# NYXFLOWER/GripNet

Hardware: NVIDIA B200
Metric: GripNet fwd+bwd edges/sec per epoch (pose-0 shape) (higher is better)
Workload: dtype f32

## Files before the change

gripnet_b200/_lib.py:

```python
import ctypes as C
import os

_HERE = os.path.dirname(os.path.abspath(__file__))
LIB_PATH = os.path.join(_HERE, "libgripnet_b200.so")


class GripnetLibraryError(RuntimeError):
    pass


class GnCsr(C.Structure):
    _fields_ = [
        ("n_rows", C.c_int32), ("n_cols", C.c_int32), ("nnz", C.c_int32), ("chunk_len", C.c_int32),
        ("n_chunks", C.c_int32), ("flags", C.c_int32),
        ("rowptr", C.c_void_p), ("col", C.c_void_p), ("val", C.c_void_p),
        ("chunk_ptr", C.c_void_p), ("chunk_row", C.c_void_p), ("chunk_beg", C.c_void_p),
        ("row_counter", C.c_void_p),
    ]


class GnAdamTensor(C.Structure):
    _fields_ = [("param", C.c_void_p), ("grad", C.c_void_p), ("exp_avg", C.c_void_p), ("exp_avg_sq", C.c_void_p),
                ("n", C.c_int64)]

# ... 5 lines not shown
class GnHaloPeer(C.Structure):
    _fields_ = [("idx", C.c_void_p), ("count", C.c_int64), ("dst_row", C.c_int64)]


class GnSumSegment(C.Structure):
    _fields_ = [("dst", C.c_void_p), ("n", C.c_int64), ("slot_offset", C.c_int64)]


_P, _I32, _I64, _F, _SZ, _INT = C.c_void_p, C.c_int32, C.c_int64, C.c_float, C.c_size_t, C.c_int
_CSR = C.POINTER(GnCsr)

SIGNATURES = {
    "gn_version": (_INT, []),
    "gn_error_string": (C.c_char_p, [_INT]),
    "gn_last_cuda_error": (_INT, []),
    "gn_last_cuda_error_string": (C.c_char_p, []),
    "gn_launch_count": (C.c_uint64, []),
    "gn_csr_from_keys_workspace_bytes": (_SZ, [_I64, _I32]),
    "gn_csr_from_keys": (_INT, [_P, _I64, _I32, _P, _P, _P, _SZ, _P]),
    "gn_rowptr_slice": (_INT, [_P, _I32, _I32, _P, _P]),
    "gn_build_chunks_workspace_bytes": (_SZ, [_I32]),
    "gn_build_chunks": (_INT, [_P, _I32, _I32, _P, _P, _P, _I64, _P, _P, _SZ, _P]),
    "gn_gcn_prep_workspace_bytes": (_SZ, [_I64, _I32, _I32]),
    "gn_gcn_prep": (_INT, [_P, _P, _P, _I64, _I32, _I32, _INT, _F, _P, _P, _P, _P, _P, _P, _P, _P, _P, _P, _P,
                           _P, _P, _P, _P, _SZ, _P]),
    "gn_edge_filter_workspace_bytes": (_SZ, [_I64]),
    "gn_edge_filter": (_INT, [_P, _P, _P, _I64, _INT, _I64, _I64, _P, _P, _P, _P, _I64, _P, _P, _SZ, _P]),
    "gn_gcn_part_workspace_bytes": (_SZ, [_I64, _I32]),
    "gn_gcn_part_structure": (_INT, [_P, _P, _P, _I64, _I32, _I32, _INT, _F, _P, _P, _P, _P, _P, _P, _P, _SZ, _P]),
    "gn_gcn_part_values": (_INT, [_P, _P, _I32, _I32, _P, _P, _INT, _P, _P]),
    "gn_rgcn_prep_workspace_bytes": (_SZ, [_I64, _I32, _I32]),
    "gn_rgcn_prep": (_INT, [_P, _P, _I64, _P, _I32, _I32, _P, _P, _P, _P, _P, _P, _P, _P, _P, _SZ, _P]),
    "gn_index_prep_workspace_bytes": (_SZ, [_I64, _I32]),
    "gn_index_prep": (_INT, [_P, _I64, _I32, _P, _P, _P, _SZ, _P]),
    "gn_spmm": (_INT, [_CSR, _P, _I64, _I32, _P, _P, _P, _I64, _INT, _P, _I64, _P, _P]),
    "gn_sgemm_workspace_bytes": (_SZ, [_I32, _I32, _I32, _I32, _INT]),
    "gn_sgemm": (_INT, [_INT, _INT, _I32, _I32, _I32, _P, _I64, _P, _I64, _P, _I64, _I32, _I64, _I64, _I64, _INT,
                        _F, _INT, _P, _I64, _P, _I64, _P, _I32, _P, _SZ, _P]),
    "gn_tc_gemm_workspace_bytes": (_SZ, [_I32, _I32, _I32]),
    "gn_tc_gemm": (_INT, [_INT, _I32, _I32, _I32, _P, _I64, _P, _I64, _P, _I64, _P, _I64, _P, _I64, _P, _SZ, _P]),
    "gn_tc_gemm_rel_workspace_bytes": (_SZ, [_I32, _I32, _I32, _I32]),
    "gn_tc_gemm_rel": (_INT, [_I32, _I32, _I32, _I32, _P, _I64, _P, _P, _I64, _P, _SZ, _P]),
    "gn_tc_rel_image": (_INT, [_I32, _I32, _I32, _I32, _P, _P, _SZ, _P]),
    "gn_tc_gemm_rel_image": (_INT, [_I32, _I32, _I32, _I32, _P, _I64, _P, _SZ, _P, _I64, _P]),
    "gn_tc_tn_workspace_bytes": (_SZ, [_I64, _I32, _I32]),
    "gn_tc_tn": (_INT, [_P, _I64, _P, _I64, _I64, _I32, _I32, _P, _I64, _I32, _I64, _P, _SZ, _P]),
    "gn_distmult_fwd": (_INT, [_P, _I64, _I32, _P, _P, _P, _P, _I64, _INT, _P, _P]),
    "gn_distmult_coef": (_INT, [_P, _P, _I64, _INT, _P, _P]),
    "gn_pair_prep_workspace_bytes": (_SZ, [_I64]),
    "gn_pair_prep": (_INT, [_P, _P, _P, _I64, _I32, _I32, _P, _P, _P, _P, _SZ, _P]),
    "gn_distmult_bwd_pairs": (_INT, [_CSR, _P, _P, _P, _P, _I64, _I32, _P, _P, _P]),
    "gn_distmult_grads_workspace_bytes": (_SZ, [_I32, _I32, _I32]),
    "gn_distmult_grads": (_INT, [_P, _P, _I32, _I32, _I32, _P, _I64, _P, _P, _I64, _P, _P, _SZ, _P]),
    "gn_softmax_fwd": (_INT, [_P, _I64, _I32, _P, _P]),
    "gn_softmax_bwd": (_INT, [_P, _P, _I64, _I32, _P, _P]),
    "gn_map2d": (_INT, [_INT, _P, _I64, _P, _I64, _I64, _I32, _P]),
    "gn_relu_bwd": (_INT, [_P, _I64, _P, _I64, _P, _I64, _I64, _I32, _P]),
    "gn_abs_bwd": (_INT, [_P, _I64, _P, _I64, _P, _I64, _I64, _I32, _F, _P]),
    "gn_axpby": (_INT, [_P, _I64, _F, _P, _I64, _F, _P, _I64, _I64, _I32, _P]),
    "gn_zero": (_INT, [_P, _SZ, _P]),
    "gn_mean3": (_INT, [_P, _I64, _P, _I64, _P, _I64, _P, _I64, _I64, _I32, _P]),
    "gn_colsum_workspace_bytes": (_SZ, [_I64, _I32]),
    "gn_colsum": (_INT, [_P, _I64, _I64, _I32, _P, _P, _SZ, _P]),
    "gn_loss_workspace_bytes": (_SZ, [_I64]),
    "gn_lp_loss_fwd": (_INT, [_P, _I64, _P, _I64, _F, _P, _P, _SZ, _P]),
    "gn_lp_loss_bwd": (_INT, [_P, _I64, _P, _I64, _F, _P, _P, _P, _P]),
    "gn_nc_loss_fwd": (_INT, [_P, _I64, _I32, _P, _F, _P, _P, _SZ, _P]),
    "gn_nc_loss_bwd": (_INT, [_P, _I64, _I32, _P, _F, _P, _P, _P]),
    "gn_negsample_table_bytes": (_SZ, [_I64]),
    "gn_negsample_build": (_INT, [_P, _P, _I64, _I64, _P, _I32, _P, _SZ, _P]),
    "gn_negsample_draw": (_INT, [_P, _SZ, _I64, _I64, _P, _I32, C.c_uint64, _P, _P, _P, _P]),
    "gn_adam_max_tensors_per_launch": (_INT, []),
    "gn_adam_step": (_INT, [_P, _I32, C.c_double, C.c_double, C.c_double, C.c_double, C.c_double, _P, _P]),
    "gn_lp_metrics_workspace_bytes": (_SZ, [_I64, _I64, _I32]),
    "gn_lp_metrics": (_INT, [_P, _I64, _P, _I64, _P, _P, _I32, _P, _P, _SZ, _P]),
    "gn_argmax_rows": (_INT, [_P, _I64, _I64, _I32, _P, _P]),
    "gn_nc_metrics_workspace_bytes": (_SZ, [_I32]),
    "gn_nc_metrics": (_INT, [_P, _P, _I64, _I32, _P, _P, _SZ, _P]),
    "gn_peer_max_world": (_INT, []),
    "gn_peer_allgather": (_INT, [_P, _I32, _I32, _I64, _I64, _I64, _I32, _P, _P, _P, _P]),
    "gn_peer_halo_grid": (_INT, []),
    "gn_peer_halo_push": (_INT, [_P, _I32, _I32, _I64, _I64, _P, _I32, _P, _I64, _I32, _P, _P, _P, _P]),
    "gn_peer_max_segments": (_INT, []),
    "gn_peer_push": (_INT, [_P, _I32, _I32, _I64, _I64, _P, _I32, _I64, _I32, _P, _P, _P, _P]),
    "gn_slot_sum": (_INT, [_P, _I32, _I64, _P, _I32, _P]),
}

GN_ERR_CUDA = -4
EW_COPY, EW_ABS, EW_RELU, EW_ADD = 0, 1, 2, 3
CSR_ROW_IS_CHUNK = 1

_lib = None


def load():
    global _lib
    if _lib is not None:
        return _lib
    if not os.path.isfile(LIB_PATH):
        raise GripnetLibraryError(
            f"{LIB_PATH} not found: build it with `python -m gripnet_b200.build` "
            "(nvcc, sm_100a).  gripnet_b200 has no CPU or PyTorch fallback.")
    try:
        lib = C.CDLL(LIB_PATH)
    except OSError as e:
        raise GripnetLibraryError(f"cannot load {LIB_PATH}: {e}") from e
# ... 19 lines not shown
```

gripnet_b200/csrc/decoder.cu:

```cuda
#include <cstdlib>

#include "rowsplit.cuh"
#include "sortkit.cuh"

namespace gn {

constexpr int kMaxNV = 8;

template <int LPE, int VEC>
__global__ void __launch_bounds__(256) distmult_fwd_kernel(const float* __restrict__ z, int64_t ldz, int D,
                                                           const float* __restrict__ w,
                                                           const int64_t* __restrict__ src,
                                                           const int64_t* __restrict__ dst,
                                                           const int64_t* __restrict__ etype, int64_t n_edges,
                                                           int sigmoid, float* __restrict__ out) {
  constexpr int EPI = 32 / LPE;
  const int lane = threadIdx.x & 31;
  const int slot = lane / LPE, fl = lane % LPE;
  const int64_t warp = (int64_t(blockIdx.x) * blockDim.x + threadIdx.x) >> 5;
  const int64_t n_warps = (int64_t(gridDim.x) * blockDim.x) >> 5;
  for (int64_t e0 = warp * EPI; e0 < n_edges; e0 += n_warps * EPI) {
    const int64_t e = e0 + slot;
    float s = 0.f;
    if (e < n_edges) {
// ... 112 lines not shown
}

template <int LPE, int VEC, int NV>
__global__ void __launch_bounds__(256) pair_walk_kernel(const gn_csr csr, const int32_t* __restrict__ ent_other,
                                                        const int32_t* __restrict__ ent_eid,
                                                        const float* __restrict__ coef, const float* __restrict__ z,
                                                        int64_t ldz, int D, float* __restrict__ T,
                                                        float* __restrict__ partial) {
  ChunkInfo ci;
  if (!chunk_info(csr, ci)) return;
  constexpr int EPI = 32 / LPE;
  const int lane = threadIdx.x & 31;
  const int slot = lane / LPE, fl = lane % LPE;
  Vec<VEC> acc[NV];
#pragma unroll
  for (int v = 0; v < NV; ++v)
#pragma unroll
    for (int i = 0; i < VEC; ++i) acc[v].v[i] = 0.f;
  for (int s0 = ci.beg + slot; s0 < ci.end; s0 += 2 * EPI) {
    const int s1 = s0 + EPI;
    const bool has1 = s1 < ci.end;
    const float* pa0 = z + int64_t(__ldg(ent_other + s0)) * ldz;
    const float* pa1 = has1 ? z + int64_t(__ldg(ent_other + s1)) * ldz : z;
    const float g0 = __ldg(coef + __ldg(ent_eid + s0));
    const float g1 = has1 ? __ldg(coef + __ldg(ent_eid + s1)) : 0.f;
    Vec<VEC> a0[NV], a1[NV];
#pragma unroll
    for (int v = 0; v < NV; ++v) {
      const int f = (v * LPE + fl) * VEC;
      if (f < D) {
        a0[v] = load_vec<VEC>(pa0 + f);
        a1[v] = load_vec<VEC>(pa1 + f);
      }
    }
#pragma unroll
    for (int v = 0; v < NV; ++v) {
      const int f = (v * LPE + fl) * VEC;
      if (f < D) {
#pragma unroll
        for (int i = 0; i < VEC; ++i) {
          acc[v].v[i] = fmaf(g0, a0[v].v[i], acc[v].v[i]);
          acc[v].v[i] = fmaf(g1, a1[v].v[i], acc[v].v[i]);
        }
      }
    }
  }
#pragma unroll
  for (int v = 0; v < NV; ++v) reduce_slots<LPE, VEC>(acc[v]);
  const int row = ci.row;
  auto emit = [&](int, int f, const Vec<VEC>& sum) { store_vec<VEC>(T + int64_t(row) * D + f, sum); };
  finish_row<LPE, VEC, NV>(csr, ci, acc, D, partial, emit);
}

template <int NV>
__global__ void __launch_bounds__(256, 4) pair_walk_batch_kernel(const gn_csr csr, const int32_t* __restrict__ ent_other,
                                                                 const int32_t* __restrict__ ent_eid,
                                                                 const float* __restrict__ coef,
                                                                 const float* __restrict__ z, int64_t ldz, int D,
                                                                 float* __restrict__ T, float* __restrict__ partial) {
  ChunkInfo ci;
  if (!chunk_info(csr, ci)) return;
  const int lane = threadIdx.x & 31;
  const int slot = lane >> 3, fl = lane & 7;
  const int D4 = D >> 2;
  const unsigned ldb = unsigned(ldz) * 4u;
  const float4* __restrict__ z4 = reinterpret_cast<const float4*>(z) + fl;
  bool ok[NV];
#pragma unroll
  for (int v = 0; v < NV; ++v) ok[v] = (v * 8 + fl) < D4;
  Vec<4> acc[NV];
#pragma unroll
  for (int v = 0; v < NV; ++v)
#pragma unroll
    for (int i = 0; i < 4; ++i) acc[v].v[i] = 0.f;
  for (int base = ci.beg; base < ci.end; base += 32) {
    const int mine = base + lane;
    int o = 0;
    float g = 0.f;
    if (mine < ci.end) {
      o = __ldg(ent_other + mine);
      g = __ldg(coef + __ldg(ent_eid + mine));
    }
    const int steps = min(8, (ci.end - base + 3) >> 2);
#pragma unroll 2
    for (int t = 0; t < steps; ++t) {
      const int from = t * 4 + slot;
      const int oo = __shfl_sync(kFull, o, from);
      const float gg = __shfl_sync(kFull, g, from);
      const float4* za = row_ptr(z4, oo, ldb);
#pragma unroll
      for (int v = 0; v < NV; ++v) {
        if (ok[v]) {
          const float4 a = __ldg(za + v * 8);
          acc[v].v[0] = fmaf(gg, a.x, acc[v].v[0]);
          acc[v].v[1] = fmaf(gg, a.y, acc[v].v[1]);
          acc[v].v[2] = fmaf(gg, a.z, acc[v].v[2]);
          acc[v].v[3] = fmaf(gg, a.w, acc[v].v[3]);
        }
      }
    }
  }
#pragma unroll
  for (int v = 0; v < NV; ++v) reduce_slots<8, 4>(acc[v]);
  const int row = ci.row;
  auto emit = [&](int, int f, const Vec<4>& sum) { store_vec<4>(T + int64_t(row) * D + f, sum); };
  finish_row<8, 4, NV>(csr, ci, acc, D, partial, emit);
}

constexpr int kGradThreads = 1024;
constexpr int kGradSlabNodes = 96;

__device__ __forceinline__ float grads_reduce_groups(float acc, int g, int G, int f, int D, float* red) {
  if (g < G && f < D) red[g * D + f] = acc;
  __syncthreads();
  float s = 0.f;
  if (g == 0 && f < D) {
    s = red[f];
    for (int k = 1; k < G; ++k) s += red[k * D + f];
  }
  __syncthreads();
  return s;
}

__global__ void __launch_bounds__(kGradThreads) distmult_grads_kernel(const float* __restrict__ T,
                                                                     const float* __restrict__ T2, int n_nodes,
                                                                     int n_rel, int D, const float* __restrict__ z,
                                                                     int64_t ldz, const float* __restrict__ w,
                                                                     float* __restrict__ dz, int64_t lddz,
                                                                     float* __restrict__ dw, int n_slabs,
                                                                     float* __restrict__ slab_part,
                                                                     unsigned int* __restrict__ slab_count) {
  extern __shared__ float red[];
  __shared__ int s_last;
  const int G = kGradThreads / D;
  const int g = int(threadIdx.x) / D, f = int(threadIdx.x) % D;
  const int n_dw_blocks = dw ? n_rel * n_slabs : 0;
  constexpr int kU = 8;
  if (int(blockIdx.x) >= n_dw_blocks) {
    const int row = int(blockIdx.x) - n_dw_blocks;
    if (dz == nullptr || row >= n_nodes) return;
    float acc = 0.f;
    if (g < G) {
      for (int i0 = g; i0 < n_rel; i0 += kU * G) {
        float tv[kU], ov[kU];
#pragma unroll
        for (int u = 0; u < kU; ++u) {
          const int i = i0 + u * G;
          tv[u] = ov[u] = 0.f;
          if (i < n_rel) {
            const int64_t t = (int64_t(row) * n_rel + i) * D + f;
            tv[u] = __ldg(T + t);
            if (T2) tv[u] += __ldg(T2 + t);
            ov[u] = __ldg(w + int64_t(i) * D + f);
          }
        }
#pragma unroll
        for (int u = 0; u < kU; ++u) acc = fmaf(tv[u], ov[u], acc);
      }
    }
// ... 397 lines not shown
  GN_PW_CASES(4, 4)
  GN_PW_CASE(8, 4, 3)
  GN_PW_CASES(32, 4)
  GN_PW_CASES(4, 1)
  GN_PW_CASES(32, 1)
#undef GN_PW_CASES
#undef GN_PW_CASE
  return GN_ERR_ARG;
}

static bool grads_vec_ok(int D, const float* T, const float* T2, const float* z, int64_t ldz, const float* w,
                         const float* dz, int64_t lddz, const float* dw) {
  return D % 4 == 0 && D <= 128 && ldz % 4 == 0 && lddz % 4 == 0 && aligned16(T) && (!T2 || aligned16(T2)) &&
         aligned16(z) && aligned16(w) && (!dz || aligned16(dz)) && (!dw || aligned16(dw));
}

size_t gn_distmult_grads_workspace_bytes(int32_t n_nodes, int32_t n_rel, int32_t D) {
  const size_t slabs = size_t(ceil_div(n_nodes > 0 ? n_nodes : 1, kGradSlabNodes));
  return align_up(size_t(n_rel > 0 ? n_rel : 1) * 4) + size_t(n_rel > 0 ? n_rel : 1) * slabs * size_t(D > 0 ? D : 1) * 4 + 256;
}

int gn_distmult_grads(const float* T, const float* T2, int32_t n_nodes, int32_t n_rel, int32_t D, const float* z,
                      int64_t ldz, const float* w, float* dz, int64_t lddz, float* dw, void* ws, size_t ws_bytes,
                      void* stream) {
  if (n_nodes <= 0 || n_rel <= 0 || D <= 0 || D > kGradThreads || !T || !z || !w || (!dz && !dw)) return GN_ERR_ARG;
  cudaStream_t st = as_stream(stream);
  const bool vec = grads_vec_ok(D, T, T2, z, ldz, w, dz, lddz, dw);
  const int n_slabs = int(ceil_div(n_nodes, vec ? kVSlab : kGradSlabNodes));
  unsigned int* count = nullptr;
  float* part = nullptr;
  if (dw && n_slabs > 1) {
    if (!ws || ws_bytes < gn_distmult_grads_workspace_bytes(n_nodes, n_rel, D)) return GN_ERR_WORKSPACE;
    count = static_cast<unsigned int*>(ws);
    part = reinterpret_cast<float*>(static_cast<char*>(ws) + align_up(size_t(n_rel) * 4));
    GN_LAUNCH(zero_u32_kernel, (unsigned)ceil_div(n_rel, 256), 256, 0, st, count, n_rel);
  }
  if (vec) {
    const int C4 = D / 4;
    const int GR = n_rel > 32 ? 8 : 1;
    const int nodes_per_cta = kVSub / GR;
    const int64_t blocks = int64_t(dw ? n_rel * n_slabs : 0) + (dz ? ceil_div(n_nodes, nodes_per_cta) : 0);
    GN_LAUNCH(distmult_grads_vec_kernel, (unsigned)blocks, C4 * kVSub, size_t(kVSub) * C4 * sizeof(float4), st, T, T2,
              n_nodes, n_rel, D, z, ldz, w, dz, lddz, dw, n_slabs, part, count, GR);
    return GN_OK;
  }
  const int G = kGradThreads / D;
  const size_t smem = size_t(G) * size_t(D) * sizeof(float);
  const int64_t blocks = int64_t(dw ? n_rel * n_slabs : 0) + (dz ? n_nodes : 0);
  GN_LAUNCH(distmult_grads_kernel, (unsigned)blocks, kGradThreads, smem, st, T, T2, n_nodes, n_rel, D, z, ldz, w, dz,
            lddz, dw, n_slabs, part, count);
  return GN_OK;
}

}
```

gripnet_b200/ops.py:

```python
import os
import weakref

import torch

from . import _lib, streams
from .graph import _ptr, _stream, _ws, require_cuda, validate_index

EPS = 1e-13


class M:
    __slots__ = ("t", "ptr", "ld", "n", "f")

    def __init__(self, t, col0=0, width=None):
        assert t.dim() == 2 and t.stride(1) == 1 and t.dtype == torch.float32
        self.t = t
        self.n = t.size(0)
        self.f = t.size(1) - col0 if width is None else width
        self.ld = t.stride(0) if t.size(0) > 1 else max(t.size(1), 1)
        self.ptr = t.data_ptr() + 4 * col0


def _as_rows(x, name):
    require_cuda(x, name)
# ... 704 lines not shown
        need = ctx.needs_input_grad[0] or ctx.needs_input_grad[1]
        br = streams.Branch()
        br_s = struct_branch if struct_branch is not None else streams.Branch(background=True)
        if need:
            with br_s(pos_index, neg_index, edge_type):
                pair_struct(neg_index, edge_type, z.size(0), r_loc)
                pair_struct(pos_index, edge_type, z.size(0), r_loc)
        with br(z, w, ni, et):
            neg = _distmult_fwd(z, w, ni, et, sigmoid)
        pos = _distmult_fwd(z, w, pi, et, sigmoid)
        br.join()
        if need and br_s._parent is None:
            ctx.struct_branch = br_s
        else:
            ctx.struct_branch = None
            br_s.join()
        ctx.sigmoid = bool(sigmoid)
        ctx.keys = (pos_index, neg_index, edge_type)
        ctx.key_versions = tuple(t._version for t in ctx.keys)
        ctx.rel = (int(rel_lo), r_loc, w_full.size(0))
        ctx.save_for_backward(z, w, pos, neg)
        return pos, neg

    @staticmethod
    def backward(ctx, g_pos, g_neg):
        from .graph import pair_struct
        z, w, pos, neg = ctx.saved_tensors
        pos_key, neg_key, et_key = ctx.keys
        _check_versions(ctx.keys, ctx.key_versions, "pos / neg edge_index or edge_type")
        rel_lo, r, r_full = ctx.rel
        n = z.size(0)
        if ctx.struct_branch is not None:
            ctx.struct_branch.join()
            ctx.struct_branch = None
        ps_p = pair_struct(pos_key, et_key, n, r)
        ps_n = pair_struct(neg_key, et_key, n, r)
        g_pos, g_neg = g_pos.contiguous(), g_neg.contiguous()
        br = streams.Branch(enabled=ps_p is not ps_n)
        with br(g_neg, neg, z):
            coef_n = _distmult_coef(g_neg, neg, ctx.sigmoid)
            t_n = _pair_walk(ps_n, coef_n, z)
        coef_p = _distmult_coef(g_pos, pos, ctx.sigmoid)
        t_p = _pair_walk(ps_p, coef_p, z)
        br.join()
        dz, dw = _distmult_grads(t_p, t_n, z, w, ctx.needs_input_grad[0], ctx.needs_input_grad[1])
        if dw is not None and r != r_full:
            dw_full = torch.empty((r_full, w.size(1)), dtype=torch.float32, device=w.device)
            _lib.check(_lib.load().gn_zero(dw_full.data_ptr(), dw_full.numel() * 4, _stream()), "gn_zero")
            map2d(_lib.EW_COPY, M(dw), M(dw_full[rel_lo: rel_lo + r]))
            dw = dw_full
        return dz, dw, None, None, None, None, None, None, None


class MultiClass(torch.autograd.Function):
    @staticmethod
    def forward(ctx, z, weight, node_list, softmax):
        lib = _lib.load()
        z = _as_rows(z, "z")
        w = _as_rows(weight, "weight").contiguous()
        require_cuda(node_list, "node_list", torch.int64)
        if w.size(0) != z.size(1):
            raise RuntimeError("decoder weight rows must equal the embedding width")
        validate_index(node_list, z.size(0), "node_list")
        idx = node_list.contiguous().view(-1)
        m, d, c = idx.numel(), z.size(1), w.size(1)
        dev = z.device
        logits = torch.empty((m, c), dtype=torch.float32, device=dev)
        sgemm(False, False, m, c, d, z.data_ptr(), z.stride(0) if z.size(0) > 1 else d, w.data_ptr(), c,
              logits.data_ptr(), c, dev, a_rows=idx)
        if softmax:
            out = torch.empty_like(logits)
            _lib.check(lib.gn_softmax_fwd(_ptr(logits), m, c, _ptr(out), _stream()), "gn_softmax_fwd")
        else:
            out = logits
        ctx.softmax = bool(softmax)
        ctx.key_tensor = node_list
        ctx.save_for_backward(z, w, out, idx)
        return out

    @staticmethod
    def backward(ctx, grad):
        from .graph import index_struct
        lib = _lib.load()
        z, w, out, idx = ctx.saved_tensors
        n, d, c, m = z.size(0), z.size(1), w.size(1), idx.numel()
        dev = z.device
        g = grad.contiguous()
        ldz = z.stride(0) if n > 1 else d
        if ctx.softmax:
            gl = torch.empty_like(g)
            _lib.check(lib.gn_softmax_bwd(_ptr(out), _ptr(g), m, c, _ptr(gl), _stream()), "gn_softmax_bwd")
        else:
            gl = g
        dz = dw = None
        if ctx.needs_input_grad[1]:
            dw = torch.empty((d, c), dtype=torch.float32, device=dev)
            sgemm(True, False, d, c, m, z.data_ptr(), ldz, gl.data_ptr(), c, dw.data_ptr(), c, dev, a_rows=idx)
        if ctx.needs_input_grad[0]:
            grows = torch.empty((max(m, 1), d), dtype=torch.float32, device=dev)
            sgemm(False, True, m, d, c, gl.data_ptr(), c, w.data_ptr(), c, grows.data_ptr(), d, dev)
            st = index_struct(ctx.key_tensor, n)
            dz = torch.empty((n, d), dtype=torch.float32, device=dev)
            spmm(st.csr, M(grows), M(dz), d)
        return dz, dw, None, None


class LinkPredLoss(torch.autograd.Function):
    @staticmethod
    def forward(ctx, pos, neg):
        lib = _lib.load()
        pos = require_cuda(pos, "pos_score", torch.float32).contiguous()
        neg = require_cuda(neg, "neg_score", torch.float32).contiguous()
        dev = pos.device
        loss = torch.empty(1, dtype=torch.float32, device=dev)
        n = max(pos.numel(), neg.numel())
        ws = _ws(lib.gn_loss_workspace_bytes(n), dev)
        _lib.check(lib.gn_lp_loss_fwd(_ptr(pos), pos.numel(), _ptr(neg), neg.numel(), EPS, _ptr(loss), _ptr(ws),
                                      ws.numel(), _stream()), "gn_lp_loss_fwd")
        ctx.save_for_backward(pos, neg)
        return loss.view(())

    @staticmethod
    def backward(ctx, grad):
        lib = _lib.load()
        pos, neg = ctx.saved_tensors
        g = grad.contiguous().view(1)
        gp, gn_ = torch.empty_like(pos), torch.empty_like(neg)
        _lib.check(lib.gn_lp_loss_bwd(_ptr(pos), pos.numel(), _ptr(neg), neg.numel(), EPS, _ptr(g), _ptr(gp),
                                      _ptr(gn_), _stream()), "gn_lp_loss_bwd")
        return gp, gn_


class NodeClassLoss(torch.autograd.Function):
    @staticmethod
    def forward(ctx, score, labels):
        lib = _lib.load()
        score = _as_rows(score, "score").contiguous()
        labels = require_cuda(labels, "labels", torch.int64).contiguous()
        if labels.numel() != score.size(0):
            raise RuntimeError("labels must have one entry per score row")
        validate_index(labels, score.size(1), "labels")
        dev = score.device
        loss = torch.empty(1, dtype=torch.float32, device=dev)
        ws = _ws(lib.gn_loss_workspace_bytes(score.size(0)), dev)
        _lib.check(lib.gn_nc_loss_fwd(_ptr(score), score.size(0), score.size(1), _ptr(labels), EPS, _ptr(loss),
                                      _ptr(ws), ws.numel(), _stream()), "gn_nc_loss_fwd")
        ctx.save_for_backward(score, labels)
        return loss.view(())

    @staticmethod
    def backward(ctx, grad):
        lib = _lib.load()
        score, labels = ctx.saved_tensors
        g = grad.contiguous().view(1)
        gs = torch.empty_like(score)
        _lib.check(lib.gn_nc_loss_bwd(_ptr(score), score.size(0), score.size(1), _ptr(labels), EPS, _ptr(g),
                                      _ptr(gs), _stream()), "gn_nc_loss_bwd")
        return gs, None


class MatMul(torch.autograd.Function):
    @staticmethod
    def forward(ctx, x, w):
        x = _as_rows(x, "x")
        w = _as_rows(w, "w").contiguous()
        out = _new(x.size(0), w.size(1), x)
        sgemm(False, False, x.size(0), w.size(1), x.size(1), x.data_ptr(), M(x).ld, w.data_ptr(), w.size(1),
              out.data_ptr(), w.size(1), x.device)
        ctx.save_for_backward(x, w)
        return out

# ... 19 lines not shown
```

gripnet_b200/pipelines.py:

```python
import os

import torch
from torch.nn import Module, Parameter

from . import parallel
from .decoder import multiClassInnerProductDecoder, multiRelaInnerProductDecoder
from . import graph as G
from . import ops, streams
from .layers import homoGraph, interGraph
from .losses import link_prediction_loss, node_classification_loss


PROLOGUE = os.environ.get("GRIPNET_B200_PROLOGUE", "1") != "0"
PREP_AT = os.environ.get("GRIPNET_B200_PREP_AT", "top")


class PoseModel(Module):
    def __init__(self, n_g, n_d, n_rel, gg=(32, 16, 16), gd=(16, 32), dd_out=32, n_base=32):
        super().__init__()
        dd = [sum(gd), dd_out]
        self.gg = homoGraph(list(gg), start_graph=True, in_dim=n_g)
        self.gd = interGraph(sum(gg), gd[0], n_d, target_feat_dim=gd[1])
        self.dd = homoGraph(dd, multi_relational=True, n_rela=n_rel, n_base=n_base)
        self.dmt = multiRelaInnerProductDecoder(sum(dd), n_rel)

    def embed(self, data, after_first=None):
        z = self.gg(None, data["gg_edge_index"], edge_weight=data.get("gg_edge_weight"), if_catout=True)
        if after_first is not None:
            after_first()
        z = self.gd(z, data["gd_edge_index"], mod="cat", if_relu=True)
        return self.dd(z, data["dd_edge_index"], edge_type=data["dd_edge_type"],
                       range_list=data["dd_range_list"], if_catout=True)

    def forward(self, data, neg_edge_index=None):
        dctx = data.get("dist")
        if dctx is not None:
            dctx.begin_step()
        if dctx is None:
            pos, et = data["dd_edge_index"], data["dd_edge_type"]
            neg = data["neg_edge_index"] if neg_edge_index is None else neg_edge_index
            n_dec = self.gd.n_target
        else:
            pos, et = data["dd_edge_index_local"], data["dd_edge_type_shifted"]
            neg = data["neg_edge_index_local"] if neg_edge_index is None else neg_edge_index
            n_dec = dctx.world * dctx.block(data["n_d_global"])
            rel_lo, rel_n = data["dd_rel_lo"], data["dd_rel_n"]
        prep = streams.Branch(background=PREP_AT == "top")

        def fork_prep():
            if torch.is_grad_enabled():
                with prep(pos, neg, et):
                    G.pair_struct(neg, et, n_dec, self.dmt.num_et if dctx is None else rel_n)
                    G.pair_struct(pos, et, n_dec, self.dmt.num_et if dctx is None else rel_n)

        def after_first():
            if PROLOGUE:
                self.dd.prologue(n_dec)
            if PREP_AT != "top":
                fork_prep()

        if PREP_AT == "top":
            fork_prep()
        z = self.embed(data, after_first=after_first)
        if dctx is None:
            pos_score, neg_score = self.dmt.score_pair(z, pos, neg, et, struct_branch=prep)
            return link_prediction_loss(pos_score, neg_score), z, pos_score, neg_score
        z_full = parallel.all_gather_rows(z, dctx, data["n_d_global"])
        pos_score, neg_score = self.dmt.score_pair(z_full, pos, neg, et, rel_lo=rel_lo, n_rel_local=rel_n,
                                                   struct_branch=prep)
        loss = parallel.global_mean_loss(link_prediction_loss(pos_score, neg_score), pos_score.numel(),
                                         data["e_dd_global"], dctx)
        return loss, z, pos_score, neg_score


class AminerModel(Module):
    def __init__(self, n_p, n_a, n_class, pp=(128, 64, 64), pa=(64, 64), aa_hid=(128, 32)):
        super().__init__()
        aa = [sum(pa)] + list(aa_hid)
        self.pp = homoGraph(list(pp), start_graph=True, in_dim=n_p)
        self.pa = interGraph(sum(pp), pa[0], n_a, target_feat_dim=pa[1])
        self.aa = homoGraph(aa)
        self.mcip = multiClassInnerProductDecoder(sum(aa), n_class)

    def forward(self, data):
        z = self.pp(None, data["pp_edge_index"], edge_weight=data.get("pp_edge_weight"), if_catout=True)
        z = self.pa(z, data["pa_edge_index"], if_relu=True, mod="cat")
        z = self.aa(z, data["aa_edge_index"], edge_weight=data.get("aa_edge_weight"), if_catout=True)
        score = self.mcip(z, data["train_node_idx"])
        return node_classification_loss(score, data["train_node_class"]), z, score


class FreebaseDModel(Module):
    def __init__(self, n_p, n_q, n_a, n_class, pp=(256, 128, 128), pa=(128, 128), aa_out=32):
        super().__init__()
        self.pp = homoGraph(list(pp), start_graph=True, in_dim=n_p)
        self.pa = interGraph(sum(pp), pa[0], n_a, target_feat_dim=pa[1], if_one_external=False)
        self.qq = homoGraph(list(pp), start_graph=True, in_dim=n_q)
        self.qa = interGraph(sum(pp), pa[0], n_a, target_feat_dim=pa[1], if_one_external=False)
        self.aa_embeddings = Parameter(torch.randn(n_a, pa[1]))
        self.aa = homoGraph([pa[1], aa_out])
        self.mcip = multiClassInnerProductDecoder(aa_out, n_class)

    def forward(self, data):
        z = self.pa(self.pp(None, data["pp_edge_index"], if_catout=True), data["pa_edge_index"], mod="add",
                    if_relu=True)
        z1 = self.qa(self.qq(None, data["qq_edge_index"], if_catout=True), data["qa_edge_index"], mod="add",
                     if_relu=True)
        z = self.aa(ops.mean3(z, z1, self.aa_embeddings), data["aa_edge_index"])
        score = self.mcip(z, data["train_node_idx"])
        return node_classification_loss(score, data["train_node_class"]), z, score


class ChainModel(Module):

    def __init__(self, n_a, n_b, n_c, n_class, hid=64, out=32):
        super().__init__()
        self.aa = homoGraph([hid, hid, hid], start_graph=True, in_dim=n_a)
# ... 126 lines not shown
```

include/gripnet_b200.h:

```cpp
#ifndef GRIPNET_B200_H
#define GRIPNET_B200_H

#include <stddef.h>
#include <stdint.h>

#ifdef __cplusplus
extern "C" {
#endif

typedef enum {
  GN_OK = 0,
  GN_ERR_ARG = -1,
  GN_ERR_RANGE = -2,
  GN_ERR_WORKSPACE = -3,
  GN_ERR_CUDA = -4
} gn_status;

int gn_version(void);
const char* gn_error_string(int status);
int gn_last_cuda_error(void);
const char* gn_last_cuda_error_string(void);
uint64_t gn_launch_count(void);

typedef struct {
// ... 54 lines not shown
int gn_rgcn_prep(const int64_t* src, const int64_t* dst, int64_t n_edges,
                 const int64_t* range_list , int32_t n_nodes, int32_t n_rel,
                 int32_t* rowptr, int32_t* col, int32_t* perm, float* inv_cnt ,
                 int32_t* rowptr_t , int32_t* col_t, float* val_t, int32_t* perm_t,
                 void* ws, size_t ws_bytes, void* stream);

size_t gn_index_prep_workspace_bytes(int64_t n, int32_t n_nodes);
int gn_index_prep(const int64_t* index, int64_t n, int32_t n_nodes,
                  int32_t* rowptr, int32_t* perm, void* ws, size_t ws_bytes, void* stream);

int gn_spmm(const gn_csr* csr, const float* x, int64_t ldx, int32_t F,
            const float* row_scale, const float* bias, const float* addend, int64_t ld_addend,
            int relu, float* out, int64_t ldo, float* partial, void* stream);

size_t gn_sgemm_workspace_bytes(int32_t M, int32_t N, int32_t K, int32_t batch, int batch_reduce);
int gn_sgemm(int transA, int transB, int32_t M, int32_t N, int32_t K,
             const float* A, int64_t lda, const float* B, int64_t ldb, float* C, int64_t ldc,
             int32_t batch, int64_t strideA, int64_t strideB, int64_t strideC, int batch_reduce,
             float alpha, int accumulate, const float* addend, int64_t ld_addend,
             const float* relu_mask, int64_t ld_mask, const int64_t* a_rows,
             int32_t split_k, float* ws, size_t ws_bytes, void* stream);

size_t gn_tc_gemm_workspace_bytes(int32_t M, int32_t N, int32_t K);
int gn_tc_gemm(int transB, int32_t M, int32_t N, int32_t K, const float* A, int64_t lda,
               const float* B, int64_t ldb, float* C, int64_t ldc,
               const float* addend, int64_t ld_addend, const float* relu_mask, int64_t ld_mask,
               void* ws, size_t ws_bytes, void* stream);

size_t gn_tc_gemm_rel_workspace_bytes(int32_t M, int32_t n_rel, int32_t f, int32_t K);
int gn_tc_gemm_rel(int32_t M, int32_t n_rel, int32_t f, int32_t K, const float* X, int64_t ldx,
                   const float* W, float* Y, int64_t ldy, void* ws, size_t ws_bytes, void* stream);
int gn_tc_rel_image(int32_t M, int32_t n_rel, int32_t f, int32_t K, const float* W, void* ws, size_t ws_bytes,
                    void* stream);
int gn_tc_gemm_rel_image(int32_t M, int32_t n_rel, int32_t f, int32_t K, const float* X, int64_t ldx,
                         const void* image, size_t image_bytes, float* Y, int64_t ldy, void* stream);

size_t gn_tc_tn_workspace_bytes(int64_t n, int32_t Mo, int32_t No);
int gn_tc_tn(const float* A, int64_t lda, const float* B, int64_t ldb, int64_t n, int32_t Mo, int32_t No,
             float* C, int64_t ldc, int32_t c_inner, int64_t c_stride, void* ws, size_t ws_bytes, void* stream);

int gn_distmult_fwd(const float* z, int64_t ldz, int32_t D, const float* w,
                    const int64_t* src, const int64_t* dst, const int64_t* etype, int64_t n_edges,
                    int sigmoid, float* out, void* stream);
int gn_distmult_coef(const float* grad_out, const float* out, int64_t n_edges, int sigmoid,
                     float* coef, void* stream);
size_t gn_pair_prep_workspace_bytes(int64_t n_edges);
int gn_pair_prep(const int64_t* src, const int64_t* dst, const int64_t* etype, int64_t n_edges, int32_t n_nodes,
                 int32_t n_rel, int32_t* pair_rowptr, int32_t* ent_other, int32_t* ent_eid ,
                 void* ws, size_t ws_bytes, void* stream);
int gn_distmult_bwd_pairs(const gn_csr* pair_csr, const int32_t* ent_other, const int32_t* ent_eid,
                          const float* coef, const float* z, int64_t ldz, int32_t D, float* T, float* partial,
                          void* stream);
size_t gn_distmult_grads_workspace_bytes(int32_t n_nodes, int32_t n_rel, int32_t D);
int gn_distmult_grads(const float* T, const float* T2 , int32_t n_nodes, int32_t n_rel, int32_t D,
                      const float* z, int64_t ldz, const float* w, float* dz , int64_t lddz,
                      float* dw , void* ws, size_t ws_bytes, void* stream);

int gn_softmax_fwd(const float* logits, int64_t n, int32_t C, float* out, void* stream);
int gn_softmax_bwd(const float* out, const float* grad_out, int64_t n, int32_t C, float* grad_logits,
                   void* stream);

enum { GN_EW_COPY = 0, GN_EW_ABS = 1, GN_EW_RELU = 2, GN_EW_ADD = 3  };
int gn_map2d(int op, const float* src, int64_t lds, float* dst, int64_t ldd, int64_t n, int32_t F,
             void* stream);
int gn_relu_bwd(const float* g, int64_t ldg, const float* y, int64_t ldy, float* dst, int64_t ldd,
                int64_t n, int32_t F, void* stream);
int gn_abs_bwd(const float* g, int64_t ldg, const float* t, int64_t ldt, float* dst, int64_t ldd,
               int64_t n, int32_t F, float scale, void* stream);
int gn_axpby(const float* a, int64_t lda, float alpha, const float* b, int64_t ldb, float beta,
             float* dst, int64_t ldd, int64_t n, int32_t F, void* stream);
int gn_zero(void* p, size_t bytes, void* stream);
int gn_mean3(const float* a, int64_t lda, const float* b, int64_t ldb, const float* c, int64_t ldc,
             float* dst, int64_t ldd, int64_t n, int32_t F, void* stream);
size_t gn_colsum_workspace_bytes(int64_t n, int32_t F);
int gn_colsum(const float* x, int64_t ldx, int64_t n, int32_t F, float* out, void* ws, size_t ws_bytes,
              void* stream);
size_t gn_loss_workspace_bytes(int64_t n);
int gn_lp_loss_fwd(const float* pos, int64_t n_pos, const float* neg, int64_t n_neg, float eps,
                   float* loss , void* ws, size_t ws_bytes, void* stream);
int gn_lp_loss_bwd(const float* pos, int64_t n_pos, const float* neg, int64_t n_neg, float eps,
                   const float* grad_loss , float* grad_pos, float* grad_neg, void* stream);
int gn_nc_loss_fwd(const float* score, int64_t n, int32_t C, const int64_t* label, float eps,
                   float* loss , void* ws, size_t ws_bytes, void* stream);
int gn_nc_loss_bwd(const float* score, int64_t n, int32_t C, const int64_t* label, float eps,
                   const float* grad_loss , float* grad_score, void* stream);

size_t gn_negsample_table_bytes(int64_t n_edges);
int gn_negsample_build(const int64_t* src, const int64_t* dst, int64_t n_edges, int64_t n_nodes,
                       const int64_t* range_list, int32_t n_rel, void* table, size_t table_bytes, void* stream);
int gn_negsample_draw(const void* table, size_t table_bytes, int64_t n_edges, int64_t n_nodes,
                      const int64_t* range_list, int32_t n_rel, uint64_t seed, uint64_t* state,
                      int64_t* neg_src, int64_t* neg_dst, void* stream);

typedef struct {
  float* param;
  const float* grad;
  float* exp_avg;
  float* exp_avg_sq;
  int64_t n;
} gn_adam_tensor;
int gn_adam_max_tensors_per_launch(void);
int gn_adam_step(const gn_adam_tensor* tensors , int32_t n_tensors, double lr, double beta1, double beta2,
                 double eps, double weight_decay, uint64_t* step, void* stream);

size_t gn_lp_metrics_workspace_bytes(int64_t n_pos, int64_t n_neg, int32_t n_rel);
int gn_lp_metrics(const float* pos_score, int64_t n_pos, const float* neg_score, int64_t n_neg,
// ... 48 lines not shown
```

Baseline: 12.12 billion.

## Fuse link-prediction loss backward into DistMult pair-walk for pos and neg

Adds a combined autograd path for the DistMult decoder plus link-prediction loss. In backward, the loss gradient and the sigmoid coefficient are computed inline per entry inside the pair-walk kernel. Positive and negative lists are handled in a single launch, which removes the separate loss-backward, coef and two walk launches along with their intermediate buffers. It applies only when rows are dense enough (a heuristic threshold). It also adds an alt_ref path so the pos and neg walks do not share a row counter, which adds API complexity.

Result: slower. 11.79 billion (median of 6 runs) (-2.8%).

```diff
diff --git a/gripnet_b200/_lib.py b/gripnet_b200/_lib.py
--- a/gripnet_b200/_lib.py
+++ b/gripnet_b200/_lib.py
@@ -81,6 +81,8 @@
     "gn_distmult_bwd_pairs": (_INT, [_CSR, _P, _P, _P, _P, _I64, _I32, _P, _P, _P]),
     "gn_distmult_grads_workspace_bytes": (_SZ, [_I32, _I32, _I32]),
     "gn_distmult_grads": (_INT, [_P, _P, _I32, _I32, _I32, _P, _I64, _P, _P, _I64, _P, _P, _SZ, _P]),
+    "gn_distmult_pair_lp_walk": (_INT, [_CSR, _P, _P, _P, _I64, _P, _P, _CSR, _P, _P, _P, _I64, _P, _P, _P, _F, _P,
+                                        _I64, _I32, _P]),
     "gn_softmax_fwd": (_INT, [_P, _I64, _I32, _P, _P]),
     "gn_softmax_bwd": (_INT, [_P, _P, _I64, _I32, _P, _P]),
     "gn_map2d": (_INT, [_INT, _P, _I64, _P, _I64, _I64, _I32, _P]),
diff --git a/gripnet_b200/csrc/decoder.cu b/gripnet_b200/csrc/decoder.cu
--- a/gripnet_b200/csrc/decoder.cu
+++ b/gripnet_b200/csrc/decoder.cu
@@ -188,6 +188,59 @@
   finish_row<LPE, VEC, NV>(csr, ci, acc, D, partial, emit);
 }
 
+template <int NV, typename Coef>
+__device__ __forceinline__ void pair_walk_batch_chunk(const gn_csr& csr, const ChunkInfo& ci,
+                                                      const int32_t* __restrict__ ent_other,
+                                                      const int32_t* __restrict__ ent_eid, Coef coef_of,
+                                                      const float* __restrict__ z, int64_t ldz, int D,
+                                                      float* __restrict__ T, float* __restrict__ partial) {
+  const int lane = threadIdx.x & 31;
+  const int slot = lane >> 3, fl = lane & 7;
+  const int D4 = D >> 2;
+  const unsigned ldb = unsigned(ldz) * 4u;
+  const float4* __restrict__ z4 = reinterpret_cast<const float4*>(z) + fl;
+  bool ok[NV];
+#pragma unroll
+  for (int v = 0; v < NV; ++v) ok[v] = (v * 8 + fl) < D4;
+  Vec<4> acc[NV];
+#pragma unroll
+  for (int v = 0; v < NV; ++v)
+#pragma unroll
+    for (int i = 0; i < 4; ++i) acc[v].v[i] = 0.f;
+  for (int base = ci.beg; base < ci.end; base += 32) {
+    const int mine = base + lane;
+    int o = 0;
+    float g = 0.f;
+    if (mine < ci.end) {
+      o = __ldg(ent_other + mine);
+      g = coef_of(__ldg(ent_eid + mine));
+    }
+    const int steps = min(8, (ci.end - base + 3) >> 2);
+#pragma unroll 2
+    for (int t = 0; t < steps; ++t) {
+      const int from = t * 4 + slot;
+      const int oo = __shfl_sync(kFull, o, from);
+      const float gg = __shfl_sync(kFull, g, from);
+      const float4* za = row_ptr(z4, oo, ldb);
+#pragma unroll
+      for (int v = 0; v < NV; ++v) {
+        if (ok[v]) {
+          const float4 a = __ldg(za + v * 8);
+          acc[v].v[0] = fmaf(gg, a.x, acc[v].v[0]);
+          acc[v].v[1] = fmaf(gg, a.y, acc[v].v[1]);
+          acc[v].v[2] = fmaf(gg, a.z, acc[v].v[2]);
+          acc[v].v[3] = fmaf(gg, a.w, acc[v].v[3]);
+        }
+      }
+    }
+  }
+#pragma unroll
+  for (int v = 0; v < NV; ++v) reduce_slots<8, 4>(acc[v]);
+  const int row = ci.row;
+  auto emit = [&](int, int f, const Vec<4>& sum) { store_vec<4>(T + int64_t(row) * D + f, sum); };
+  finish_row<8, 4, NV>(csr, ci, acc, D, partial, emit);
+}
+
 template <int NV>
 __global__ void __launch_bounds__(256, 4) pair_walk_batch_kernel(const gn_csr csr, const int32_t* __restrict__ ent_other,
                                                                  const int32_t* __restrict__ ent_eid,
@@ -196,51 +249,43 @@
                                                                  float* __restrict__ T, float* __restrict__ partial) {
   ChunkInfo ci;
   if (!chunk_info(csr, ci)) return;
-  const int lane = threadIdx.x & 31;
-  const int slot = lane >> 3, fl = lane & 7;
-  const int D4 = D >> 2;
-  const unsigned ldb = unsigned(ldz) * 4u;
-  const float4* __restrict__ z4 = reinterpret_cast<const float4*>(z) + fl;
-  bool ok[NV];
-#pragma unroll
-  for (int v = 0; v < NV; ++v) ok[v] = (v * 8 + fl) < D4;
-  Vec<4> acc[NV];
-#pragma unroll
-  for (int v = 0; v < NV; ++v)
-#pragma unroll
-    for (int i = 0; i < 4; ++i) acc[v].v[i] = 0.f;
-  for (int base = ci.beg; base < ci.end; base += 32) {
-    const int mine = base + lane;
-    int o = 0;
-    float g = 0.f;
-    if (mine < ci.end) {
-      o = __ldg(ent_other + mine);
-      g = __ldg(coef + __ldg(ent_eid + mine));
-    }
-    const int steps = min(8, (ci.end - base + 3) >> 2);
-#pragma unroll 2
-    for (int t = 0; t < steps; ++t) {
-      const int from = t * 4 + slot;
-      const int oo = __shfl_sync(kFull, o, from);
-      const float gg = __shfl_sync(kFull, g, from);
-      const float4* za = row_ptr(z4, oo, ldb);
-#pragma unroll
-      for (int v = 0; v < NV; ++v) {
-        if (ok[v]) {
-          const float4 a = __ldg(za + v * 8);
-          acc[v].v[0] = fmaf(gg, a.x, acc[v].v[0]);
-          acc[v].v[1] = fmaf(gg, a.y, acc[v].v[1]);
-          acc[v].v[2] = fmaf(gg, a.z, acc[v].v[2]);
-          acc[v].v[3] = fmaf(gg, a.w, acc[v].v[3]);
-        }
-      }
-    }
-  }
-#pragma unroll
-  for (int v = 0; v < NV; ++v) reduce_slots<8, 4>(acc[v]);
-  const int row = ci.row;
-  auto emit = [&](int, int f, const Vec<4>& sum) { store_vec<4>(T + int64_t(row) * D + f, sum); };
-  finish_row<8, 4, NV>(csr, ci, acc, D, partial, emit);
+  pair_walk_batch_chunk<NV>(csr, ci, ent_other, ent_eid, [&](int e) { return __ldg(coef + e); }, z, ldz, D, T,
+                            partial);
+}
+
+struct LpWalkList {
+  gn_csr csr;
+  const int32_t* ent_other;
+  const int32_t* ent_eid;
+  const float* score;
+  int64_t n;
+  float* T;
+  float* partial;
+};
+
+template <int NV, bool NEG>
+__device__ __forceinline__ void pair_walk_lp_list(const LpWalkList& L, int warp, float g, float eps,
+                                                  const float* __restrict__ z, int64_t ldz, int D) {
+  ChunkInfo ci;
+  if (!chunk_info_at(L.csr, warp, ci)) return;
+  const float fn = float(L.n);
+  const float* __restrict__ score = L.score;
+  auto coef_of = [&](int e) {
+    const float p = __ldg(score + e);
+    const float gl = NEG ? g / (fn * (1.0f - p + eps)) : -g / (fn * (p + eps));
+    return gl * (p * (1.0f - p));
+  };
+  pair_walk_batch_chunk<NV>(L.csr, ci, L.ent_other, L.ent_eid, coef_of, z, ldz, D, L.T, L.partial);
+}
+
+template <int NV>
+__global__ void __launch_bounds__(256, 4) pair_walk_lp_kernel(const LpWalkList pos, const LpWalkList neg,
+                                                              const float* __restrict__ grad_loss, float eps,
+                                                              const float* __restrict__ z, int64_t ldz, int D) {
+  const int warp = int((int64_t(blockIdx.x) * blockDim.x + threadIdx.x) >> 5);
+  const float g = __ldg(grad_loss);
+  if (warp < pos.csr.n_chunks) pair_walk_lp_list<NV, false>(pos, warp, g, eps, z, ldz, D);
+  else pair_walk_lp_list<NV, true>(neg, warp - pos.csr.n_chunks, g, eps, z, ldz, D);
 }
 
 constexpr int kGradThreads = 1024;
@@ -744,4 +789,39 @@
   return GN_OK;
 }
 
-}
+int gn_distmult_pair_lp_walk(const gn_csr* pos_csr, const int32_t* pos_other, const int32_t* pos_eid,
+                             const float* pos_score, int64_t n_pos, float* T_pos, float* pos_partial,
+                             const gn_csr* neg_csr, const int32_t* neg_other, const int32_t* neg_eid,
+                             const float* neg_score, int64_t n_neg, float* T_neg, float* neg_partial,
+                             const float* grad_loss, float eps, const float* z, int64_t ldz, int32_t D, void* stream) {
+  if (!pos_csr || !neg_csr || !grad_loss || !z || !T_pos || !T_neg) return GN_ERR_ARG;
+  if (D <= 0 || D > 128 || D % 4 != 0 || ldz % 4 != 0 || ldz >= (int64_t(1) << 30)) return GN_ERR_ARG;
+  if (!aligned16(z) || !aligned16(T_pos) || !aligned16(T_neg)) return GN_ERR_ARG;
+  if ((pos_partial && !aligned16(pos_partial)) || (neg_partial && !aligned16(neg_partial))) return GN_ERR_ARG;
+  if (pos_csr->row_counter == neg_csr->row_counter && pos_csr->n_chunks > 0) return GN_ERR_ARG;
+  const LpWalkList lists[2] = {
+      {*pos_csr, pos_other, pos_eid, pos_score, n_pos, T_pos, pos_partial},
+      {*neg_csr, neg_other, neg_eid, neg_score, n_neg, T_neg, neg_partial}};
+  for (const LpWalkList& L : lists) {
+    if (L.csr.nnz > 0 && (!L.ent_other || !L.ent_eid || !L.score)) return GN_ERR_ARG;
+    if (L.csr.n_chunks > L.csr.n_rows && !L.partial) return GN_ERR_ARG;
+  }
+  const int64_t chunks = int64_t(pos_csr->n_chunks) + neg_csr->n_chunks;
+  if (chunks == 0) return GN_OK;
+  const int nv = (D / 4 + 7) / 8;
+  const unsigned grid = (unsigned)ceil_div(chunks, 8);
+  cudaStream_t st = as_stream(stream);
+#define GN_PLW_CASE(N)                                                                                               \
+  if (nv == N) {                                                                                                     \
+    GN_LAUNCH((pair_walk_lp_kernel<N>), grid, 256, 0, st, lists[0], lists[1], grad_loss, eps, z, ldz, D);            \
+    return GN_OK;                                                                                                    \
+  }
+  GN_PLW_CASE(1)
+  GN_PLW_CASE(2)
+  GN_PLW_CASE(3)
+  GN_PLW_CASE(4)
+#undef GN_PLW_CASE
+  return GN_ERR_ARG;
+}
+
+}
diff --git a/gripnet_b200/ops.py b/gripnet_b200/ops.py
--- a/gripnet_b200/ops.py
+++ b/gripnet_b200/ops.py
@@ -780,6 +780,104 @@
         return dz, dw, None, None, None, None, None, None, None
 
 
+DECODER_HEAD_SPLIT = os.environ.get("GRIPNET_B200_DECODER_HEAD") == "split"
+
+
+_LP_HEAD_MIN_ROW_ENTRIES = 48
+
+
+def lp_head_fusable(z, n_rel, n_edges):
+    if DECODER_HEAD_SPLIT or os.environ.get("GRIPNET_B200_DECODER_KERNELS", "").startswith("l"):
+        return False
+    d, ldz = z.size(1), _ldz(z)
+    return (n_edges > 0 and 2 * n_edges >= _LP_HEAD_MIN_ROW_ENTRIES * z.size(0) * n_rel and d % 4 == 0 and d <= 128
+            and ldz % 4 == 0 and ldz < (1 << 30) and z.data_ptr() % 16 == 0)
+
+
+def _lp_loss(pos, neg):
+    lib = _lib.load()
+    loss = torch.empty(1, dtype=torch.float32, device=pos.device)
+    ws = _ws(lib.gn_loss_workspace_bytes(max(pos.numel(), neg.numel())), pos.device)
+    _lib.check(lib.gn_lp_loss_fwd(_ptr(pos), pos.numel(), _ptr(neg), neg.numel(), EPS, _ptr(loss), _ptr(ws),
+                                  ws.numel(), _stream()), "gn_lp_loss_fwd")
+    return loss
+
+
+class DistMultPairLPLoss(torch.autograd.Function):
+
+    @staticmethod
+    def forward(ctx, z, weight, pos_index, neg_index, edge_type, struct_branch=None):
+        from .graph import pair_struct
+        z, w, pi, et = _distmult_check(z, weight, pos_index, edge_type)
+        _, _, ni, _ = _distmult_check(z, w, neg_index, edge_type)
+        r = w.size(0)
+        need = ctx.needs_input_grad[0] or ctx.needs_input_grad[1]
+        br = streams.Branch()
+        br_s = struct_branch if struct_branch is not None else streams.Branch(background=True)
+        if need:
+            with br_s(pos_index, neg_index, edge_type):
+                pair_struct(neg_index, edge_type, z.size(0), r)
+                pair_struct(pos_index, edge_type, z.size(0), r)
+        with br(z, w, ni, et):
+            neg = _distmult_fwd(z, w, ni, et, True)
+        pos = _distmult_fwd(z, w, pi, et, True)
+        br.join()
+        loss = _lp_loss(pos, neg)
+        if need and br_s._parent is None:
+            ctx.struct_branch = br_s
+        else:
+            ctx.struct_branch = None
+            br_s.join()
+        ctx.set_materialize_grads(False)
+        ctx.keys = (pos_index, neg_index, edge_type)
+        ctx.key_versions = tuple(t._version for t in ctx.keys)
+        ctx.save_for_backward(z, w, pos, neg)
+        return loss.view(()), pos, neg
+
+    @staticmethod
+    def backward(ctx, g_loss, g_pos, g_neg):
+        from .graph import pair_struct
+        lib = _lib.load()
+        z, w, pos, neg = ctx.saved_tensors
+        pos_key, neg_key, et_key = ctx.keys
+        _check_versions(ctx.keys, ctx.key_versions, "pos / neg edge_index or edge_type")
+        if ctx.struct_branch is not None:
+            ctx.struct_branch.join()
+            ctx.struct_branch = None
+        need_z, need_w = ctx.needs_input_grad[0], ctx.needs_input_grad[1]
+        if g_loss is None and g_pos is None and g_neg is None:
+            return None, None, None, None, None, None
+        n, d, e = z.size(0), z.size(1), pos.numel()
+        ps_p = pair_struct(pos_key, et_key, n, w.size(0))
+        ps_n = pair_struct(neg_key, et_key, n, w.size(0))
+        if g_pos is None and g_neg is None:
+            t_p = torch.empty((ps_p.csr.n_rows, d), dtype=torch.float32, device=z.device)
+            t_n = torch.empty((ps_n.csr.n_rows, d), dtype=torch.float32, device=z.device)
+            part_p, part_n = ps_p.csr.partial(d), ps_n.csr.partial(d)
+            neg_ref = ps_n.csr.alt_ref() if ps_n is ps_p else ps_n.csr.ref
+            g = g_loss.contiguous().view(1)
+            _lib.check(lib.gn_distmult_pair_lp_walk(
+                ps_p.csr.ref, _ptr(ps_p.ent_other), _ptr(ps_p.ent_eid), _ptr(pos), e, _ptr(t_p), _ptr(part_p),
+                neg_ref, _ptr(ps_n.ent_other), _ptr(ps_n.ent_eid), _ptr(neg), e, _ptr(t_n), _ptr(part_n),
+                _ptr(g), EPS, z.data_ptr(), _ldz(z), d, _stream()), "gn_distmult_pair_lp_walk")
+        else:
+            gp, gn_ = torch.empty_like(pos), torch.empty_like(neg)
+            if g_loss is not None:
+                _lib.check(lib.gn_lp_loss_bwd(_ptr(pos), e, _ptr(neg), e, EPS, _ptr(g_loss.contiguous().view(1)),
+                                              _ptr(gp), _ptr(gn_), _stream()), "gn_lp_loss_bwd")
+            for acc, g in ((gp, g_pos), (gn_, g_neg)):
+                if g_loss is None and g is None:
+                    _lib.check(lib.gn_zero(acc.data_ptr(), acc.numel() * 4, _stream()), "gn_zero")
+                elif g_loss is None:
+                    map2d(_lib.EW_COPY, M(g.contiguous().view(1, -1)), M(acc.view(1, -1)))
+                elif g is not None:
+                    map2d(_lib.EW_ADD, M(g.contiguous().view(1, -1)), M(acc.view(1, -1)))
+            t_n = _pair_walk(ps_n, _distmult_coef(gn_, neg, True), z)
+            t_p = _pair_walk(ps_p, _distmult_coef(gp, pos, True), z)
+        dz, dw = _distmult_grads(t_p, t_n, z, w, need_z, need_w)
+        return dz, dw, None, None, None, None
+
+
 class MultiClass(torch.autograd.Function):
     @staticmethod
     def forward(ctx, z, weight, node_list, softmax):
@@ -836,15 +934,9 @@
 class LinkPredLoss(torch.autograd.Function):
     @staticmethod
     def forward(ctx, pos, neg):
-        lib = _lib.load()
         pos = require_cuda(pos, "pos_score", torch.float32).contiguous()
         neg = require_cuda(neg, "neg_score", torch.float32).contiguous()
-        dev = pos.device
-        loss = torch.empty(1, dtype=torch.float32, device=dev)
-        n = max(pos.numel(), neg.numel())
-        ws = _ws(lib.gn_loss_workspace_bytes(n), dev)
-        _lib.check(lib.gn_lp_loss_fwd(_ptr(pos), pos.numel(), _ptr(neg), neg.numel(), EPS, _ptr(loss), _ptr(ws),
-                                      ws.numel(), _stream()), "gn_lp_loss_fwd")
+        loss = _lp_loss(pos, neg)
         ctx.save_for_backward(pos, neg)
         return loss.view(())
 
diff --git a/gripnet_b200/pipelines.py b/gripnet_b200/pipelines.py
--- a/gripnet_b200/pipelines.py
+++ b/gripnet_b200/pipelines.py
@@ -63,6 +63,9 @@
             fork_prep()
         z = self.embed(data, after_first=after_first)
         if dctx is None:
+            if ops.lp_head_fusable(z, self.dmt.num_et, et.numel()):
+                loss, pos_score, neg_score = ops.DistMultPairLPLoss.apply(z, self.dmt.weight, pos, neg, et, prep)
+                return loss, z, pos_score, neg_score
             pos_score, neg_score = self.dmt.score_pair(z, pos, neg, et, struct_branch=prep)
             return link_prediction_loss(pos_score, neg_score), z, pos_score, neg_score
         z_full = parallel.all_gather_rows(z, dctx, data["n_d_global"])
diff --git a/include/gripnet_b200.h b/include/gripnet_b200.h
--- a/include/gripnet_b200.h
+++ b/include/gripnet_b200.h
@@ -130,6 +130,12 @@
                           const float* coef, const float* z, int64_t ldz, int32_t D, float* T, float* partial,
                           void* stream);
 size_t gn_distmult_grads_workspace_bytes(int32_t n_nodes, int32_t n_rel, int32_t D);
+int gn_distmult_pair_lp_walk(const gn_csr* pos_csr, const int32_t* pos_other, const int32_t* pos_eid,
+                             const float* pos_score, int64_t n_pos, float* T_pos, float* pos_partial,
+                             const gn_csr* neg_csr, const int32_t* neg_other, const int32_t* neg_eid,
+                             const float* neg_score, int64_t n_neg, float* T_neg, float* neg_partial,
+                             const float* grad_loss , float eps, const float* z, int64_t ldz, int32_t D,
+                             void* stream);
 int gn_distmult_grads(const float* T, const float* T2 , int32_t n_nodes, int32_t n_rel, int32_t D,
                       const float* z, int64_t ldz, const float* w, float* dz , int64_t lddz,
                       float* dw , void* ws, size_t ws_bytes, void* stream);
```
